# hku-mars/loam_livox

Hardware: AMD Instinct MI355X
Metric: scans_per_s (higher is better)
Workload: dtype f32 points / f64 solve; 1 GPU; C2: 24k-pt Mid-40 scan vs 5M-pt corner+surface map, 10 ICP iters (fixed), k=5, Q-full; scan_points=24000, map_points=4975193, map_corner=995155, map_surf=3980038, icp_iters=10, distinct_scans_in_batch=256

## Files before the change

### loam_livox_amd/build.py

```python
from __future__ import annotations

import os
import shutil
import subprocess
import sys

HERE = os.path.dirname(os.path.abspath(__file__))
CSRC = os.path.join(HERE, "csrc")
LIB = os.environ.get("LL_LIB_OUT") or os.path.join(HERE, "libloamlivox_hip.so")
SOURCES = ["ll_api_common.hip", "ll_api_fe.hip", "ll_api_map.hip", "ll_api_reg.hip", "ll_api_voxel.hip", "ll_api_cellmap.hip", "ll_api_scene_align.hip", "ll_api_keyframe_bank.hip", "ll_api_pose_graph.hip", "ll_api_history.hip", "ll_api_history_batch_buffer.hip", "ll_api_history_batch_stores.hip", "ll_api_history_batch_extract.hip", "ll_api_history_batch_cells.hip", "ll_fe_kernels.hip", "ll_map_kernels.hip", "ll_reg_query_kernels.hip", "ll_reg_solve_kernels.hip", "ll_reg_maps_kernels.hip", "ll_reg_aux_kernels.hip", "ll_reg_small_kernels.hip", "ll_knn_kernels.hip", "ll_voxel_kernels.hip", "ll_cellmap_kernels.hip", "ll_cellmap_extract_kernels.hip", "ll_cellmap_select_kernels.hip", "ll_spin_kernels.hip", "ll_spin_api.hip", "ll_history_batch_kernels.hip", "ll_cellmap_batch_kernels.hip", "ll_cellmap_batch_extract_kernels.hip", "ll_cellmatch_batch_kernels.hip", "ll_fullmap_batch_kernels.hip", "ll_keyframe_bank_kernels.hip", "ll_pose_graph_kernels.hip"]
HEADERS = ["ll_api_internal.h", "ll_api_history_batch_internal.h", "ll_device.h", "ll_fe_core.h", "ll_knn_core.h", "ll_knn_coop.h", "ll_knn_tile.h", "ll_reg_query.h", "ll_reg_solve_fast.h", "ll_reg_big_path.h", "ll_reg_solve_general.h", "ll_reg_solve_common.h", "ll_reg_small_solve.h", "ll_reg_core.h", "ll_voxel.h", "ll_voxel_core.h", "ll_cellmap.h", "ll_cellmap_core.h", "ll_cellmap_select_core.h", "ll_spin.h", "ll_spin_core.h", "ll_history_batch.h", "ll_cellmap_batch.h", "ll_cellmap_batch_core.h", "ll_cellmap_batch_extract_core.h", "ll_cellmatch_batch.h", "ll_cellmatch_batch_core.h", "ll_fullmap_batch.h", "ll_fullmap_batch_core.h", "ll_keyframe_bank.h", "ll_keyframe_bank_core.h", "ll_pose_graph.h", "ll_pose_graph_core.h", "../../include/loam_livox_hip.h"]
FLAGS = ["--offload-arch=gfx950", "-O3", "-std=c++17", "-fPIC", "-ffp-contract=off", "-Wno-unused-result"]
FLAGS += os.environ.get("LL_EXTRA_HIPCC_FLAGS", "").split()


def hipcc() -> str:
    for cand in (shutil.which("hipcc"), "/opt/rocm/bin/hipcc"):
        if cand and os.path.exists(cand):
            return cand
    raise RuntimeError("hipcc not found (ROCm toolchain required to build libloamlivox_hip.so)")



def needs_build(lib: str = LIB) -> bool:
    if not os.path.exists(lib):
        return True
    t = os.path.getmtime(lib)
    deps = [os.path.join(CSRC, f) for f in SOURCES + HEADERS] + [os.path.abspath(__file__)]
    return any(os.path.getmtime(d) > t for d in deps)


def build(force: bool = False, verbose: bool = False, lib: str = LIB, extra_flags=()) -> str:
    if not force and not needs_build(lib):
        return lib
    cc = hipcc()
    default = os.path.join(HERE, "libloamlivox_hip.so")
    objdir = os.path.join(HERE, "build" if lib == default else "build_" + os.path.basename(lib).replace(".so", ""))
    os.makedirs(objdir, exist_ok=True)
    objs = []
    procs = []
    for src in SOURCES:
        obj = os.path.join(objdir, src.replace(".hip", ".o"))
        cmd = [cc] + FLAGS + list(extra_flags) + ["-c", os.path.join(CSRC, src), "-o", obj]
        if verbose:
            print(" ".join(cmd), file=sys.stderr)
        procs.append((src, subprocess.Popen(cmd, stdout=subprocess.PIPE, stderr=subprocess.STDOUT)))
        objs.append(obj)
    for src, p in procs:
        out, _ = p.communicate()
        if p.returncode != 0:
            raise RuntimeError(f"hipcc failed on {src}:\n{out.decode()}")
        if verbose and out:
            print(out.decode(), file=sys.stderr)
    cmd = [cc, "--offload-arch=gfx950", "-shared", "-fPIC", "-o", lib] + objs
    subprocess.check_call(cmd)
    return lib


if __name__ == "__main__":
    print(build(force="--force" in sys.argv, verbose=True))
```

### loam_livox_amd/csrc/ll_reg_solve_fast.h

```cpp
#pragma once
#include <hip/hip_runtime.h>

#include "ll_reg_query.h"
#include "ll_reg_solve_common.h"

namespace ll {

#define RS_WAVES (RS_THREADS / 64)

#define LL_CTX_DECL(x)                                   \
    double R_[9], t_[3];                                  \
    MbRot mb_;                                            \
    {                                                     \
        const double q_[4] = {(x)[0], (x)[1], (x)[2], (x)[3]}; \
        quat_to_mat(q_, R_);                              \
        t_[0] = (x)[4];                                   \
        t_[1] = (x)[5];                                   \
        t_[2] = (x)[6];                                   \
        if (DEBLUR) mb_prepare(q_, mb_);                  \
    }
#define LL_CTX_ACCUM(kind, ff, a, v, huber_a, acc)                                                        \
    do {                                                                                                  \
        const double f_[3] = {(double)(ff).x, (double)(ff).y, (double)(ff).z};                            \
        if (DEBLUR)                                                                                       \
            block_accumulate_mb((kind), mb_, t_, (double)(ff).w, f_, (a), (v), (huber_a), (acc));  \
        else                                                                                              \
            block_accumulate((kind), R_, t_, f_, (a), (v), (huber_a), (acc));            \
    } while (0)
#define LL_CTX_L1(out, kind, ff, a, v, huber_a, q_last)                                                   \
    do {                                                                                                  \
        const double f_[3] = {(double)(ff).x, (double)(ff).y, (double)(ff).z};                            \
        if (DEBLUR)                                                                                       \
            (out) = block_l1_mb((kind), mb_, t_, (double)(ff).w, f_, (a), (v), (huber_a), (q_last));      \
        else                                                                                              \
            (out) = block_l1((kind), R_, t_, f_, (a), (v), (huber_a), (q_last));                          \
    } while (0)

#ifdef LL_SOLVE_TIMING
#define LL_T0(var) long long var = clock64()
#define LL_TACC(slot, var)                                   \
    do {                                                     \
        if (threadIdx.x == 0) sh.tcyc[slot] += clock64() - var; \
    } while (0)
#else
#define LL_T0(var)
#define LL_TACC(slot, var)
#endif

struct SolveShared {
    long long tcyc[16];
    LmCtl ctl;
    double red[RS_WAVES][LL_NACC];
    double sum[LL_NACC];
    int need;
    int hist[256];
    int sel_bin, sel_cnt, n_cand;
    int isum[RS_WAVES];
    unsigned long long lsum[RS_WAVES];
    unsigned long long sel_prefix;
    int sel_rank;
    int n_active, n_corner_avail, n_surf_avail, n_unique;
    int l1_valid;
    int pt_T, pt_Tl, pt_kc, pt_priv;
    double fit[10];
    int pt_nl;
    double thr;
    int grp_g, grp_G, grp_seq, grp_abort;
    int xch_seq, xch_epoch;
    unsigned int xch[LL_GRP][2 * LL_NACC];
};

#define LL_GRP_SPIN_LIMIT (1 << 22)
template <bool FULL>
__device__ __forceinline__ void group_barrier(const RegDev &rd, int b, SolveShared &sh)
{
    if (FULL) __threadfence();
    __syncthreads();
    if (threadIdx.x == 0 && !sh.grp_abort) {
        const int target = (++sh.grp_seq) * sh.grp_G;
        int *bar = rd.grp_ctl + 1 + 2 * b, *abt = bar + 1;
        __hip_atomic_fetch_add(bar, 1, __ATOMIC_RELEASE, __HIP_MEMORY_SCOPE_AGENT);
        int spins = 0;
        while (__hip_atomic_load(bar, __ATOMIC_RELAXED, __HIP_MEMORY_SCOPE_AGENT) < target) {
            if (++spins > LL_GRP_SPIN_LIMIT || ((spins & 1023) == 0 && __hip_atomic_load(abt, __ATOMIC_RELAXED, __HIP_MEMORY_SCOPE_AGENT))) {
                sh.grp_abort = 1;
                __hip_atomic_store(abt, 1, __ATOMIC_RELAXED, __HIP_MEMORY_SCOPE_AGENT);
                break;
            }
        }
        if (!sh.grp_abort && __hip_atomic_load(abt, __ATOMIC_RELAXED, __HIP_MEMORY_SCOPE_AGENT)) sh.grp_abort = 1;
    }
    __syncthreads();
    if (FULL) __threadfence();
}

template <bool FULL>
__device__ __forceinline__ void group_reduce(const RegDev &rd, int b, SolveShared &sh)
{
    const int tid = threadIdx.x, G = sh.grp_G;
    if (FULL) {
        double *part = rd.grp_part + ((size_t)b * 2 + (sh.grp_seq & 1)) * LL_GRP * LL_NACC;
        if (tid < LL_NACC) __hip_atomic_store(part + sh.grp_g * LL_NACC + tid, sh.sum[tid], __ATOMIC_RELAXED, __HIP_MEMORY_SCOPE_AGENT);
        group_barrier<true>(rd, b, sh);
        if (tid < LL_NACC) {
            double t = 0.0;
            for (int k = 0; k < G; k++) t += __hip_atomic_load(part + k * LL_NACC + tid, __ATOMIC_RELAXED, __HIP_MEMORY_SCOPE_AGENT);
            sh.sum[tid] = t;
        }
        __syncthreads();
        return;
    }
    constexpr int NG = 2 * LL_NACC;
    static_assert(LL_GRP * NG <= RS_THREADS, "one polling thread per granule");
    if (tid == 0) sh.xch_seq++;
    __syncthreads();
    const int seq = sh.xch_seq;
    if (!sh.grp_abort && seq < 4096) {
        const unsigned int tag = ((unsigned int)sh.xch_epoch << 12) | (unsigned int)seq;
        unsigned long long *slot = rd.grp_xch + ((size_t)b * 2 + (seq & 1)) * LL_GRP * NG;
        if (tid < NG) {
            const unsigned long long bits = (unsigned long long)__double_as_longlong(sh.sum[tid >> 1]);
            const unsigned int half = (tid & 1) ? (unsigned int)(bits >> 32) : (unsigned int)bits;
            __hip_atomic_store(slot + sh.grp_g * NG + tid, ((unsigned long long)tag << 32) | (unsigned long long)half, __ATOMIC_RELAXED,
                               __HIP_MEMORY_SCOPE_AGENT);
        }
        if (tid < G * NG) {
            const int *abt = rd.grp_ctl + 2 + 2 * b;
            unsigned long long v = __hip_atomic_load(slot + tid, __ATOMIC_RELAXED, __HIP_MEMORY_SCOPE_AGENT);
            int spins = 0;
            while ((unsigned int)(v >> 32) != tag) {
                if (++spins > LL_GRP_SPIN_LIMIT || ((spins & 1023) == 0 && __hip_atomic_load(abt, __ATOMIC_RELAXED, __HIP_MEMORY_SCOPE_AGENT))) {
                    sh.grp_abort = 1;
                    __hip_atomic_store(const_cast<int *>(abt), 1, __ATOMIC_RELAXED, __HIP_MEMORY_SCOPE_AGENT);
                    break;
                }
                __builtin_amdgcn_s_sleep(1);
                v = __hip_atomic_load(slot + tid, __ATOMIC_RELAXED, __HIP_MEMORY_SCOPE_AGENT);
            }
            sh.xch[tid / NG][tid % NG] = (unsigned int)v;
        }
    } else if (tid == 0 && !sh.grp_abort) {
        sh.grp_abort = 1;
        __hip_atomic_store(rd.grp_ctl + 2 + 2 * b, 1, __ATOMIC_RELAXED, __HIP_MEMORY_SCOPE_AGENT);
    }
    __syncthreads();
    if (tid < LL_NACC && !sh.grp_abort) {
        double t = 0.0;
        for (int k = 0; k < G; k++)
            t += __longlong_as_double((long long)(((unsigned long long)sh.xch[k][2 * tid + 1] << 32) | (unsigned long long)sh.xch[k][2 * tid]));
        sh.sum[tid] = t;
    }
    __syncthreads();
}

__device__ __forceinline__ unsigned long long block_sum_u64(unsigned long long v, SolveShared &sh)
{
    const int tid = threadIdx.x, lane = tid & 63, wave = tid >> 6;
#pragma unroll
    for (int off = 32; off > 0; off >>= 1) v += (unsigned long long)__shfl_down((long long)v, off);
    if (lane == 0) sh.lsum[wave] = v;
    __syncthreads();
    unsigned long long s = 0;
    for (int w = 0; w < RS_WAVES; w++) s += sh.lsum[w];
    __syncthreads();
    return s;
}

__device__ int block_sum_int(int v, SolveShared &sh)
{
    const int tid = threadIdx.x, lane = tid & 63, wave = tid >> 6;
#pragma unroll
    for (int off = 32; off > 0; off >>= 1) v += __shfl_down(v, off);
    if (lane == 0) sh.isum[wave] = v;
    __syncthreads();
    int s = 0;
    for (int w = 0; w < RS_WAVES; w++) s += sh.isum[w];
    __syncthreads();
    return s;
}

__device__ __forceinline__ unsigned long long hash64(unsigned long long k)
{
    k ^= k >> 33;
    k *= 0xff51afd7ed558ccdull;
    k ^= k >> 33;
    k *= 0xc4ceb9fe1a85ec53ull;
    k ^= k >> 33;
    return k;
}



#define FAST_MAXK (FAST_MAX_BLOCKS / RS_THREADS)
#define HASH_EMPTY 0xffffffffffffffffull
#define HT_SIZE 16384
#define HT_PART 6144
#define DD2_WORDS 16384
#define DD2_SLOTS (DD2_WORDS * 16)
#define DD2B_WORDS 8192
#define DD2B_SLOTS (DD2B_WORDS * 16)
#define DD2_LIST 2048
#define SEL_BINS 4096
#define SEL_CAND 1024


template <int NK>
__device__ __forceinline__ void inlier_threshold_regs(const double (&l1r)[NK], int total, unsigned long long *s_table, SolveShared &sh,
                                                      const RegConst &rc)
{
    static_assert(NK <= 64 && NK <= FAST_MAXK, "register tile of the fast paths (one bit per entry in the 64-bit masks)");
    const int tid = threadIdx.x;
    LL_T0(t_dd);
    unsigned long long first_mask = 0;
    {
        int my = 0;
        unsigned int *bmA = (unsigned int *)s_table;
        unsigned int *bmB = bmA + DD2_WORDS;
        unsigned long long *dl = (unsigned long long *)(bmB + DD2B_WORDS);
        {
            uint4 *z = (uint4 *)s_table;
            for (int e = tid; e < (DD2_WORDS + DD2B_WORDS) / 4; e += RS_THREADS) z[e] = make_uint4(0u, 0u, 0u, 0u);
            if (tid == 0) sh.n_cand = 0;
        }
        __syncthreads();
        const int kt = (total + RS_THREADS - 1) / RS_THREADS;
        auto slot_a = [](unsigned long long key) -> unsigned int {
            unsigned int h = (unsigned int)key * 0x9E3779B1u;
            h ^= h >> 15;
            h += (unsigned int)(key >> 32) * 0x85EBCA77u;
            h ^= h >> 13;
            return h & (DD2_SLOTS - 1);
        };
        auto slot_b = [](unsigned long long key) -> unsigned int {
            unsigned int h2 = ((unsigned int)(key >> 32) * 0xC2B2AE3Du) ^ ((unsigned int)key * 0x27D4EB2Fu);
            return (h2 ^ (h2 >> 16)) & (DD2B_SLOTS - 1);
        };
        unsigned long long valid_mask = 0, cont_mask = 0;
#pragma unroll
        for (int k = 0; k < NK; k++) {
            if (k >= kt) continue;
            const double l1 = l1r[k];
            const bool valid = l1 >= 0.0;
            const unsigned int slot = slot_a((unsigned long long)__double_as_longlong(l1));
            const unsigned int bit0 = valid ? (1u << ((slot & 15u) * 2u)) : 0u;
            const unsigned int old = atomicOr(&bmA[slot >> 4], bit0);
            atomicOr(&bmA[slot >> 4], (old & bit0) << 1);
            if (valid) valid_mask |= 1ull << k;
        }
        __syncthreads();
#pragma unroll
        for (int k = 0; k < NK; k++) {
            if (k >= kt) continue;
            const unsigned long long key = (unsigned long long)__double_as_longlong(l1r[k]);
            const unsigned int slot = slot_a(key);
            const bool contested = ((valid_mask >> k) & 1ull) && ((bmA[slot >> 4] >> ((slot & 15u) * 2u)) & 2u);
            const unsigned int h2 = slot_b(key);
            const unsigned int bit0 = contested ? (1u << ((h2 & 15u) * 2u)) : 0u;
            const unsigned int old = atomicOr(&bmB[h2 >> 4], bit0);
            atomicOr(&bmB[h2 >> 4], (old & bit0) << 1);
            if (contested) cont_mask |= 1ull << k;
        }
        __syncthreads();
        unsigned long long twice_mask = 0;
#pragma unroll
        for (int k = 0; k < NK; k++) {
            if (k >= kt) continue;
            const unsigned int h2 = slot_b((unsigned long long)__double_as_longlong(l1r[k]));
            if (((cont_mask >> k) & 1ull) && ((bmB[h2 >> 4] >> ((h2 & 15u) * 2u)) & 2u)) twice_mask |= 1ull << k;
        }
        my = __popcll(valid_mask & ~twice_mask);
        first_mask = valid_mask & ~twice_mask;
        int my_pos[2] = {-1, -1};
        int n_twice = __popcll(twice_mask);
        if (twice_mask) {
            int got = 0;
#pragma unroll
            for (int k = 0; k < NK; k++) {
                if (!((twice_mask >> k) & 1ull)) continue;
                const int pos = atomicAdd(&sh.n_cand, 1);
                if (pos < DD2_LIST) dl[pos] = (unsigned long long)__double_as_longlong(l1r[k]);
                if (got < 2) my_pos[got] = pos;
                got++;
            }
        }
        const int over = block_sum_int(n_twice > 2 ? 1 : 0, sh);
        const int n_list = sh.n_cand;
        if (n_list <= DD2_LIST && over == 0) {
            if (twice_mask) {
                int got = 0;
#pragma unroll
                for (int k = 0; k < NK; k++) {
                    if (!((twice_mask >> k) & 1ull)) continue;
                    const int pos = my_pos[got < 2 ? got : 1];
                    got++;
                    const unsigned long long key = (unsigned long long)__double_as_longlong(l1r[k]);
                    bool dup = false;
                    for (int j = 0; j < pos; j++) dup |= (dl[j] == key);
                    if (!dup) {
                        first_mask |= 1ull << k;
                        my++;
                    }
                }
            }
        } else {
            first_mask = 0;
            my = 0;
            const int rounds = (total + HT_PART - 1) / HT_PART;
            for (int rnd = 0; rnd < rounds; rnd++) {
                __syncthreads();
                for (int e = tid; e < HT_SIZE; e += RS_THREADS) s_table[e] = HASH_EMPTY;
                __syncthreads();
#pragma unroll
                for (int k = 0; k < NK; k++) {
                    const double l1 = l1r[k];
                    if (!(l1 >= 0.0)) continue;
                    const unsigned long long key = (unsigned long long)__double_as_longlong(l1);
                    const unsigned long long hk = hash64(key);
                    if ((int)((hk >> 40) % (unsigned long long)rounds) != rnd) continue;
                    unsigned int h = (unsigned int)hk & (HT_SIZE - 1);
                    for (;;) {
                        const unsigned long long old = atomicCAS(&s_table[h], HASH_EMPTY, key);
                        if (old == HASH_EMPTY) {
                            first_mask |= (1ull << k);
                            my++;
                            break;
                        }
                        if (old == key) break;
                        h = (h + 1u) & (HT_SIZE - 1);
                    }
                }
            }
        }
        const int nu = block_sum_int(my, sh);
        if (tid == 0) {
            sh.n_unique = nu;
            sh.sel_prefix = 0ull;
            int target = (int)(rc.inlier_ratio * (double)nu);
            if (target > nu - 1) target = nu - 1;
            sh.sel_rank = target;
        }
        __syncthreads();
    }
    LL_TACC(3, t_dd);
    LL_T0(t_sel);
    if (sh.n_unique > 0) {
        int *bins = (int *)s_table;
        unsigned long long *cand = s_table + SEL_BINS / 2;
        double kmin = INFINITY, kmax = -INFINITY;
#pragma unroll
        for (int k = 0; k < NK; k++)
            if (first_mask & (1ull << k)) {
                kmin = fmin(kmin, l1r[k]);
                kmax = fmax(kmax, l1r[k]);
            }
        for (int off = 32; off > 0; off >>= 1) {
            kmin = fmin(kmin, __shfl_down(kmin, off));
            kmax = fmax(kmax, __shfl_down(kmax, off));
        }
        if ((tid & 63) == 0) {
            sh.red[tid >> 6][0] = kmin;
            sh.red[tid >> 6][1] = kmax;
        }
        for (int e = tid; e < SEL_BINS; e += RS_THREADS) bins[e] = 0;
        __syncthreads();
        double lo = sh.red[0][0], hi = sh.red[0][1];
        for (int w = 1; w < RS_WAVES; w++) {
            lo = fmin(lo, sh.red[w][0]);
            hi = fmax(hi, sh.red[w][1]);
        }
        const double scale = (hi > lo) ? (double)(SEL_BINS - 1) / (hi - lo) : 0.0;
#pragma unroll
        for (int k = 0; k < NK; k++)
            if (first_mask & (1ull << k)) {
                int bi = (int)((l1r[k] - lo) * scale);
                bi = bi < 0 ? 0 : (bi > SEL_BINS - 1 ? SEL_BINS - 1 : bi);
                atomicAdd(&bins[bi], 1);
            }
        __syncthreads();
        {
            const int per = SEL_BINS / RS_THREADS;
            const int lane = tid & 63, wave = tid >> 6;
            int part = 0;
            for (int e = 0; e < per; e++) part += bins[tid * per + e];
            int incl = part;
#pragma unroll
            for (int off = 1; off < 64; off <<= 1) {
                const int y = __shfl_up(incl, off);
                if (lane >= off) incl += y;
            }
            if (lane == 63) sh.isum[wave] = incl;
            if (tid == 0) sh.n_cand = 0;
            __syncthreads();
            int below = incl - part;
            for (int w = 0; w < wave; w++) below += sh.isum[w];
            const int rank = sh.sel_rank;
            __syncthreads();
            const bool last_thread = tid == RS_THREADS - 1;
            if ((rank >= below && rank < below + part) || (last_thread && rank >= below + part)) {
                int cum = below, bi = tid * per;
                for (; bi < tid * per + per - 1; bi++) {
                    if (cum + bins[bi] > rank) break;
                    cum += bins[bi];
                }
                sh.sel_bin = bi;
                sh.sel_rank = rank - cum;
                sh.sel_cnt = bins[bi];
            }
            __syncthreads();
        }
        if (sh.sel_cnt <= SEL_CAND) {
            const int sel_bin = sh.sel_bin;
#pragma unroll
            for (int k = 0; k < NK; k++)
                if (first_mask & (1ull << k)) {
                    int bi = (int)((l1r[k] - lo) * scale);
                    bi = bi < 0 ? 0 : (bi > SEL_BINS - 1 ? SEL_BINS - 1 : bi);
                    if (bi == sel_bin) cand[atomicAdd(&sh.n_cand, 1)] = (unsigned long long)__double_as_longlong(l1r[k]);
                }
            __syncthreads();
            const int m = sh.n_cand;
            for (int i = tid; i < m; i += RS_THREADS) {
                const unsigned long long ki = cand[i];
                int rk = 0;
                for (int j = 0; j < m; j++) rk += (cand[j] < ki) ? 1 : 0;
                if (rk == sh.sel_rank) sh.sel_prefix = ki;
            }
            __syncthreads();
        } else {
            const int sel_bin = sh.sel_bin;
            if (tid == 0) sh.sel_prefix = 0ull;
            __syncthreads();
            for (int pass = 0; pass < 8; pass++) {
                const int shift = 56 - 8 * pass;
                for (int e = tid; e < 256; e += RS_THREADS) sh.hist[e] = 0;
                __syncthreads();
                const unsigned long long prefix = sh.sel_prefix;
#pragma unroll
                for (int k = 0; k < NK; k++) {
                    if (!(first_mask & (1ull << k))) continue;
                    int bi = (int)((l1r[k] - lo) * scale);
                    bi = bi < 0 ? 0 : (bi > SEL_BINS - 1 ? SEL_BINS - 1 : bi);
                    if (bi != sel_bin) continue;
                    const unsigned long long key = (unsigned long long)__double_as_longlong(l1r[k]);
                    if (pass == 0 || (key >> (shift + 8)) == prefix) atomicAdd(&sh.hist[(int)((key >> shift) & 255ull)], 1);
                }
                __syncthreads();
                if (tid == 0) {
                    int rank = sh.sel_rank, d = 0, cum = 0;
                    for (d = 0; d < 256; d++) {
                        if (cum + sh.hist[d] > rank) break;
                        cum += sh.hist[d];
                    }
                    if (d > 255) d = 255;
                    sh.sel_rank = rank - cum;
                    sh.sel_prefix = (prefix << 8) | (unsigned long long)d;
                }
                __syncthreads();
            }
        }
        if (tid == 0) sh.thr = fmax(rc.inliner_dis, __longlong_as_double((long long)sh.sel_prefix));
    } else {
        if (tid == 0) sh.thr = rc.inliner_dis;
    }
    __syncthreads();
    LL_TACC(4, t_sel);
}

struct BlkRegs {
    float4 f;
    double a0, a1, a2, v0, v1, v2;
};

__device__ __forceinline__ void load_blk(const RegDev &rd, size_t sb, const double *av, int slot, BlkRegs &r)
{
    r.f = gload_f4(rd.blk_f + sb + slot);
    av_load(av, rd.cap, slot, slot < rd.cap_c, r.a0, r.a1, r.a2, r.v0, r.v1, r.v2);
}


#define PT_SLOTS 8192
#define PT_MAX_PROBE 192
#define PT_LDS_BYTES 155648
#define PT_TCAP (PT_LDS_BYTES / 32)
#define LL_LINE_CACHE_MAX 1024
#define PT_EMPTY_A 0xffffffffffffffffull
#define PT_EMPTY_B 0xffffffffu
#define PT_PRIVATE 0xffffu
#define PT_INACTIVE 0xfffeu
#define PT_NTRIP (FAST_MAX_BLOCKS / RS_THREADS / 8)

struct PtSlot {
    unsigned long long a;
    unsigned int b;
    unsigned int id;
};

__device__ __forceinline__ unsigned short gload_u16(const unsigned short *p) { return *(const LL_AS_GLOBAL unsigned short *)p; }

__device__ __forceinline__ unsigned int pt_hash(unsigned int p0, unsigned int p1, unsigned int p2)
{
    unsigned int h = p0 * 0x9E3779B1u;
    h ^= h >> 15;
    h += p1 * 0x85EBCA77u;
    h ^= h >> 13;
    h += p2 * 0xC2B2AE3Du;
    h ^= h >> 16;
    return h;
}

template <int MAX_PROBE = PT_MAX_PROBE>
__device__ __forceinline__ unsigned int pt_insert(LL_AS_LDS PtSlot *ht, unsigned int p0, unsigned int p1, unsigned int p2)
{
    const unsigned long long A = ((unsigned long long)p0 << 32) | (unsigned long long)p1;
    const unsigned int hh = pt_hash(p0, p1, p2);
    unsigned int h = hh & (PT_SLOTS - 1);
    const unsigned int step = ((hh >> 13) | 1u) & (PT_SLOTS - 1);
    for (int probe = 0; probe < MAX_PROBE; probe++) {
        unsigned long long a = __hip_atomic_load(&ht[h].a, __ATOMIC_RELAXED, __HIP_MEMORY_SCOPE_WORKGROUP);
        unsigned int bb = __hip_atomic_load(&ht[h].b, __ATOMIC_RELAXED, __HIP_MEMORY_SCOPE_WORKGROUP);
        if (a == A && bb == p2) return h;
        if (a == PT_EMPTY_A) {
            if (__hip_atomic_compare_exchange_strong(&ht[h].a, &a, A, __ATOMIC_RELAXED, __ATOMIC_RELAXED, __HIP_MEMORY_SCOPE_WORKGROUP)) a = A;
        }
        if (a == A) {
            if (bb == PT_EMPTY_B) {
                if (__hip_atomic_compare_exchange_strong(&ht[h].b, &bb, p2, __ATOMIC_RELAXED, __ATOMIC_RELAXED, __HIP_MEMORY_SCOPE_WORKGROUP)) bb = p2;
            }
            if (bb == p2) return h;
        }
        h = (h + step) & (PT_SLOTS - 1);
    }
    return PT_PRIVATE;
}

template <bool SCALED = false>
__device__ __forceinline__ void pt_plane(const f4 *map_pts, const double *pose_last, unsigned int i0, unsigned int i1, unsigned int i2, int4 &ob, int4 &oc)
{
    const f4 m0 = gload_pt(map_pts + i0), m1 = gload_pt(map_pts + i1), m2 = gload_pt(map_pts + i2);
    const double pa[3] = {(double)m0.x, (double)m0.y, (double)m0.z};
    const double pb[3] = {(double)m1.x, (double)m1.y, (double)m1.z};
    const double pc[3] = {(double)m2.x, (double)m2.y, (double)m2.z};
    double a_out[3] = {0.0, 0.0, 0.0}, v_out[3] = {0.0, 0.0, 0.0};
    (void)block_plane(pose_last, pa, pb, pc, a_out, v_out);
    if (SCALED) {
        double m_[3], beta_;
        plane_scale(v_out, a_out[0], m_, &beta_);
        v_out[0] = m_[0], v_out[1] = m_[1], v_out[2] = m_[2], a_out[0] = beta_;
    }
    ob = make_int4(__double2loint(v_out[0]), __double2hiint(v_out[0]), __double2loint(v_out[1]), __double2hiint(v_out[1]));
    oc = make_int4(__double2loint(v_out[2]), __double2hiint(v_out[2]), __double2loint(a_out[0]), __double2hiint(a_out[0]));
}

__device__ __forceinline__ int4 *pt_table_global(const RegDev &rd, int b, int g, bool grouped)
{
    return rd.pl_tab + ((size_t)b * rd.tab_cap + (grouped ? (size_t)g * (rd.tab_cap / LL_GRP) : 0)) * 2;
}

#define PT_MAP_OFF (PT_SLOTS * 16)
template <bool GROUPED>
__device__ __noinline__ unsigned long long census_and_plane_table(const RegDev &rd, const RegConst &rc, const f4 *map_pts, int b, const RegState *st,
                                                                  int nC, int nS, uint4 *s_raw, SolveShared &sh)
{
    const int tid = threadIdx.x, lane = tid & 63, wave = tid >> 6;
    constexpr int G = GROUPED ? LL_GRP : 1, GS = G * RS_THREADS;
    const int g = GROUPED ? sh.grp_g : 0;
    const int p0 = g * RS_THREADS + tid;
// ... 538 lines not shown
        }
        __syncthreads();
        LL_TACC(1, t1);
    }
}

template <int NK, bool GROUPED>
__device__ __noinline__ unsigned long long inlier_phase3(const RegDev &rd, const RegConst &rc, int b, RegState *st, SolveShared &sh, uint4 *s_raw,
                                                         unsigned long long act, int nC, int nS)
{
    constexpr int DEBLUR = 0;
    const int tid = threadIdx.x;
    const int nSp = (nS + RS_THREADS - 1) / RS_THREADS * RS_THREADS;
    const int totp = nSp + nC;
    const size_t sb = (size_t)b * rd.cap;
    LL_T0(t_l1);
    double *l1g = rd.blk_l1 + sb;
    if (!sh.l1_valid) {
        LL_CTX_DECL(sh.ctl.x)
        constexpr int G = GROUPED ? LL_GRP : 1, GS = G * RS_THREADS;
        const int g = GROUPED ? sh.grp_g : 0;
        const int p0 = g * RS_THREADS + tid;
        const int4 *tabG = pt_table_global(rd, b, g, GROUPED);
        const unsigned short *ids = rd.blk_id + (size_t)b * rd.cap_s;
        const float4 *feat = rd.surf_feat + (size_t)b * rd.feat_stride_s;
        const double *av = rd.blk_av + (size_t)b * 6 * rd.cap;
        int k = 0;
        for (int p = p0; p < nS; p += GS, k++) {
            if (!((act >> (g + G * k)) & 1ull)) continue;
            const float4 ff = gload_f4(feat + p);
            const unsigned int id = gload_u16(ids + p);
            const int4 qb = gload_i4(tabG + 2 * id), qc = gload_i4(tabG + 2 * id + 1);
            const double f[3] = {(double)ff.x, (double)ff.y, (double)ff.z};
            const double v[3] = {__hiloint2double(qb.y, qb.x), __hiloint2double(qb.w, qb.z), __hiloint2double(qc.y, qc.x)};
            l1g[rd.cap_c + p] = plane_l1_scaled(R_, t_, f, v, __hiloint2double(qc.w, qc.z), rc.huber_a, st->pose_last);
        }
        const int kpl = nSp / RS_THREADS;
        k = 0;
        for (int l = p0; l < nC; l += GS, k++) {
            if (!((act >> (kpl + g + G * k)) & 1ull)) continue;
            BlkRegs br;
            load_blk(rd, sb, av, l, br);
            const double a[3] = {br.a0, br.a1, br.a2};
            const double v[3] = {br.v0, br.v1, br.v2};
            double l1;
            LL_CTX_L1(l1, BLK_LINE, br.f, a, v, rc.huber_a, st->pose_last);
            l1g[l] = l1;
        }
        if (GROUPED)
            group_barrier<true>(rd, b, sh);
        else
            __syncthreads();
    } else if (tid == 0) {
        sh.tcyc[9] += 1;
    }
    double l1r[NK];
    {
        const int kt = (totp + RS_THREADS - 1) / RS_THREADS;
#pragma unroll
        for (int k = 0; k < NK; k++) {
            const int j = tid + k * RS_THREADS;
            double v = -1.0;
            if (k < kt) {
                const int jc = j < totp ? j : 0;
                const size_t src = jc < nS ? (size_t)rd.cap_c + jc : (jc >= nSp ? (size_t)(jc - nSp) : (size_t)rd.cap_c);
                v = gload_f64(l1g + src);
            }
            l1r[k] = v;
        }
#pragma unroll
        for (int k = 0; k < NK; k++) l1r[k] = ((act >> k) & 1ull) ? l1r[k] : -1.0;
    }
    __syncthreads();
    LL_TACC(2, t_l1);

    inlier_threshold_regs<NK>(l1r, totp, (unsigned long long *)s_raw, sh, rc);

    LL_T0(t_prune);
    {
        const double thr = sh.thr;
        int na = 0;
#pragma unroll
        for (int k = 0; k < NK; k++) {
            if (!((act >> k) & 1ull)) continue;
            if (l1r[k] > thr)
                act &= ~(1ull << k);
            else
                na++;
        }
        na = block_sum_int(na, sh);
        if (tid == 0) sh.n_active = na;
        __syncthreads();
    }
    LL_TACC(7, t_prune);
    return act;
}

template <bool GROUPED>
__device__ void solve_fast3(const RegDev &rd, const RegConst &rc, const f4 *map_pts, int b, RegState *st, SolveShared &sh, uint4 *s_raw)
{
    constexpr int DEBLUR = 0;
    const int tid = threadIdx.x;
    const int nC = rd.n_corner[b], nS = rd.n_surf[b];
    const int nSp = (nS + RS_THREADS - 1) / RS_THREADS * RS_THREADS;
    const int totp = nSp + nC;
    const size_t sb = (size_t)b * rd.cap;
    if (tid < 16) sh.tcyc[tid] = 0;
    __syncthreads();
    LL_T0(t_total);

    unsigned long long act = census_and_plane_table<GROUPED>(rd, rc, map_pts, b, st, nC, nS, s_raw, sh);

    solver_lm3<true, GROUPED>(rd, rc, b, nC, nS, st->inc, rc.ceres_prerun_times, sh.n_active, act, s_raw, st->pose_last, sh);
    int lm_iters = sh.ctl.iteration;

    if (totp <= 36 * RS_THREADS)
        act = inlier_phase3<36, GROUPED>(rd, rc, b, st, sh, s_raw, act, nC, nS);
    else
        act = inlier_phase3<FAST_MAXK, GROUPED>(rd, rc, b, st, sh, s_raw, act, nC, nS);

    {
        __shared__ double x_start_3[7];
        if (tid < 7) x_start_3[tid] = sh.ctl.x[tid];
        plane_table_reload(rd, b, GROUPED, s_raw, sh);
        solver_lm3<false, GROUPED>(rd, rc, b, nC, nS, x_start_3, rc.ceres_max_iterations, sh.n_active, act, s_raw, st->pose_last, sh);
    }
    lm_iters += sh.ctl.iteration;
    if (GROUPED) {
        group_barrier<false>(rd, b, sh);
        if (sh.grp_g != 0) return;
        if (sh.grp_abort) {
            if (tid == 0) {
                st->aborted = 1;
                st->done = 1;
                st->icp_iters += 1;
            }
            return;
        }
    }
    solve_epilogue(rc, st, sh, lm_iters);
#ifdef LL_SOLVE_TIMING
    LL_TACC(5, t_total);
    if (tid == 0)
        for (int i = 0; i < 16; i++) st->dbg_cycles[i] += sh.tcyc[i];
#endif
}

struct SolveTicket {
    int b, g, G;
};
__device__ __forceinline__ SolveTicket solve_fast_ticket(const RegDev &rd, const RegConst &rc, SolveShared &sh)
{
    SolveTicket t = {(int)blockIdx.x, 0, 1};
    if (rc.solve_group > 1) {
        if (threadIdx.x == 0) sh.grp_seq = atomicAdd(rd.grp_ctl, 1);
        __syncthreads();
        t.G = rc.solve_group;
        t.b = sh.grp_seq / t.G;
        t.g = sh.grp_seq - t.b * t.G;
        __syncthreads();
    }
    return t;
}
__device__ __forceinline__ bool solve_fast_check(const RegDev &rd, const RegConst &rc, int b, int g, int nC, int nS, RegState *st)
{
    if (padded_block_count(nC, nS) > FAST_MAX_BLOCKS || !scan_is_compact(rd, rc, b)) {
        if (g == 0 && threadIdx.x == 0) {
            st->aborted = 1;
            st->done = 1;
            st->icp_iters += 1;
        }
// ... 19 lines not shown
```

Baseline: 52620 scans/s.

## Fuse inlier histogram build into dedup pass and batch LDS atomics branchlessly

Computes the min/max range before de-duplication and builds the selection histogram during the first slot-table pass, subtracting duplicates afterward instead of re-binning unique values in a separate pass. This removes a reduction, a zeroing pass and several block barriers. The dedup and candidate-gather loops are restructured into batches of independent LDS atomics with dummy no-op targets so the divergent branches become predicated code, and the per-thread twice-list handling is simplified. The histogram range now covers duplicate values too, and the extra no-op atomics add LDS traffic.

```diff
diff --git a/loam_livox_amd/build.py b/loam_livox_amd/build.py
--- a/loam_livox_amd/build.py
+++ b/loam_livox_amd/build.py
@@ -9,7 +9,7 @@
 CSRC = os.path.join(HERE, "csrc")
 LIB = os.environ.get("LL_LIB_OUT") or os.path.join(HERE, "libloamlivox_hip.so")
 SOURCES = ["ll_api_common.hip", "ll_api_fe.hip", "ll_api_map.hip", "ll_api_reg.hip", "ll_api_voxel.hip", "ll_api_cellmap.hip", "ll_api_scene_align.hip", "ll_api_keyframe_bank.hip", "ll_api_pose_graph.hip", "ll_api_history.hip", "ll_api_history_batch_buffer.hip", "ll_api_history_batch_stores.hip", "ll_api_history_batch_extract.hip", "ll_api_history_batch_cells.hip", "ll_fe_kernels.hip", "ll_map_kernels.hip", "ll_reg_query_kernels.hip", "ll_reg_solve_kernels.hip", "ll_reg_maps_kernels.hip", "ll_reg_aux_kernels.hip", "ll_reg_small_kernels.hip", "ll_knn_kernels.hip", "ll_voxel_kernels.hip", "ll_cellmap_kernels.hip", "ll_cellmap_extract_kernels.hip", "ll_cellmap_select_kernels.hip", "ll_spin_kernels.hip", "ll_spin_api.hip", "ll_history_batch_kernels.hip", "ll_cellmap_batch_kernels.hip", "ll_cellmap_batch_extract_kernels.hip", "ll_cellmatch_batch_kernels.hip", "ll_fullmap_batch_kernels.hip", "ll_keyframe_bank_kernels.hip", "ll_pose_graph_kernels.hip"]
-HEADERS = ["ll_api_internal.h", "ll_api_history_batch_internal.h", "ll_device.h", "ll_fe_core.h", "ll_knn_core.h", "ll_knn_coop.h", "ll_knn_tile.h", "ll_reg_query.h", "ll_reg_solve_fast.h", "ll_reg_big_path.h", "ll_reg_solve_general.h", "ll_reg_solve_common.h", "ll_reg_small_solve.h", "ll_reg_core.h", "ll_voxel.h", "ll_voxel_core.h", "ll_cellmap.h", "ll_cellmap_core.h", "ll_cellmap_select_core.h", "ll_spin.h", "ll_spin_core.h", "ll_history_batch.h", "ll_cellmap_batch.h", "ll_cellmap_batch_core.h", "ll_cellmap_batch_extract_core.h", "ll_cellmatch_batch.h", "ll_cellmatch_batch_core.h", "ll_fullmap_batch.h", "ll_fullmap_batch_core.h", "ll_keyframe_bank.h", "ll_keyframe_bank_core.h", "ll_pose_graph.h", "ll_pose_graph_core.h", "../../include/loam_livox_hip.h"]
+HEADERS = ["ll_api_internal.h", "ll_api_history_batch_internal.h", "ll_device.h", "ll_fe_core.h", "ll_knn_core.h", "ll_knn_coop.h", "ll_knn_tile.h", "ll_reg_query.h", "ll_reg_solve_fast.h", "ll_reg_big_path.h", "ll_reg_solve_general.h", "ll_reg_solve_common.h", "ll_inlier_slots.h", "ll_reg_small_solve.h", "ll_reg_core.h", "ll_voxel.h", "ll_voxel_core.h", "ll_cellmap.h", "ll_cellmap_core.h", "ll_cellmap_select_core.h", "ll_spin.h", "ll_spin_core.h", "ll_history_batch.h", "ll_cellmap_batch.h", "ll_cellmap_batch_core.h", "ll_cellmap_batch_extract_core.h", "ll_cellmatch_batch.h", "ll_cellmatch_batch_core.h", "ll_fullmap_batch.h", "ll_fullmap_batch_core.h", "ll_keyframe_bank.h", "ll_keyframe_bank_core.h", "ll_pose_graph.h", "ll_pose_graph_core.h", "../../include/loam_livox_hip.h"]
 FLAGS = ["--offload-arch=gfx950", "-O3", "-std=c++17", "-fPIC", "-ffp-contract=off", "-Wno-unused-result"]
 FLAGS += os.environ.get("LL_EXTRA_HIPCC_FLAGS", "").split()
 
diff --git a/loam_livox_amd/csrc/ll_inlier_slots.h b/loam_livox_amd/csrc/ll_inlier_slots.h
--- /dev/null
+++ b/loam_livox_amd/csrc/ll_inlier_slots.h
@@ -0,0 +1,55 @@
+#pragma once
+#include <stdint.h>
+
+#ifndef LL_HD
+#if defined(__HIPCC__)
+#define LL_HD __host__ __device__ __forceinline__
+#else
+#define LL_HD inline
+#endif
+#endif
+
+namespace ll {
+
+#define DD2_WORDS 16384
+#define DD2_SLOTS (DD2_WORDS * 16)
+#define DD2B_WORDS 8192
+#define DD2B_SLOTS (DD2B_WORDS * 16)
+#define DD2_LIST_CAP 2048
+#define SEL_BINS 4096
+#define SEL_CAND 1024
+
+LL_HD unsigned int dd2_slot_a(unsigned long long key)
+{
+    unsigned int h = (unsigned int)key * 0x9E3779B1u;
+    h ^= h >> 15;
+    h += (unsigned int)(key >> 32) * 0x85EBCA77u;
+    h ^= h >> 13;
+    return h & (DD2_SLOTS - 1);
+}
+
+LL_HD unsigned int dd2_slot_b(unsigned long long key)
+{
+    const unsigned int h2 = ((unsigned int)(key >> 32) * 0xC2B2AE3Du) ^ ((unsigned int)key * 0x27D4EB2Fu);
+    return (h2 ^ (h2 >> 16)) & (DD2B_SLOTS - 1);
+}
+
+LL_HD unsigned int dd2_word(unsigned int slot) { return slot >> 4; }
+LL_HD unsigned int dd2_shift(unsigned int slot) { return (slot & 15u) * 2u; }
+LL_HD unsigned int dd2_first(unsigned int slot, bool takes_part) { return takes_part ? (1u << dd2_shift(slot)) : 0u; }
+LL_HD unsigned int dd2_second(unsigned int old_word, unsigned int first) { return (old_word & first) << 1; }
+LL_HD bool dd2_contested(unsigned int word, unsigned int slot) { return ((word >> dd2_shift(slot)) & 2u) != 0u; }
+
+LL_HD double sel_scale(double lo, double hi) { return (hi > lo) ? (double)(SEL_BINS - 1) / (hi - lo) : 0.0; }
+LL_HD int sel_bin_of(double v, double lo, double scale)
+{
+    const int bi = (int)((v - lo) * scale);
+    return bi < 0 ? 0 : (bi > SEL_BINS - 1 ? SEL_BINS - 1 : bi);
+}
+LL_HD int sel_target_rank(double ratio, int n_distinct)
+{
+    const int target = (int)(ratio * (double)n_distinct);
+    return target > n_distinct - 1 ? n_distinct - 1 : target;
+}
+
+}
diff --git a/loam_livox_amd/csrc/ll_reg_solve_fast.h b/loam_livox_amd/csrc/ll_reg_solve_fast.h
--- a/loam_livox_amd/csrc/ll_reg_solve_fast.h
+++ b/loam_livox_amd/csrc/ll_reg_solve_fast.h
@@ -1,6 +1,7 @@
 #pragma once
 #include <hip/hip_runtime.h>
 
+#include "ll_inlier_slots.h"
 #include "ll_reg_query.h"
 #include "ll_reg_solve_common.h"
 
@@ -55,6 +56,7 @@
     int need;
     int hist[256];
     int sel_bin, sel_cnt, n_cand;
+    int dd_over;
     int isum[RS_WAVES];
     unsigned long long lsum[RS_WAVES];
     unsigned long long sel_prefix;
@@ -166,7 +168,7 @@
     return s;
 }
 
-__device__ int block_sum_int(int v, SolveShared &sh)
+__device__ __forceinline__ int block_sum_int_inl(int v, SolveShared &sh)
 {
     const int tid = threadIdx.x, lane = tid & 63, wave = tid >> 6;
 #pragma unroll
@@ -178,6 +180,8 @@
     __syncthreads();
     return s;
 }
+
+__device__ int block_sum_int(int v, SolveShared &sh) { return block_sum_int_inl(v, sh); }
 
 __device__ __forceinline__ unsigned long long hash64(unsigned long long k)
 {
@@ -195,13 +199,10 @@
 #define HASH_EMPTY 0xffffffffffffffffull
 #define HT_SIZE 16384
 #define HT_PART 6144
-#define DD2_WORDS 16384
-#define DD2_SLOTS (DD2_WORDS * 16)
-#define DD2B_WORDS 8192
-#define DD2B_SLOTS (DD2B_WORDS * 16)
 #define DD2_LIST 2048
-#define SEL_BINS 4096
-#define SEL_CAND 1024
+static_assert(DD2_LIST == DD2_LIST_CAP, "the list capacity the host protocol is run with");
+#define DD2_BATCH 12
+#define SEL_BINS_OFF (HT_SIZE * 8)
 
 
 template <int NK>
@@ -212,93 +213,150 @@
     const int tid = threadIdx.x;
     LL_T0(t_dd);
     unsigned long long first_mask = 0;
+    int *bins = (int *)((char *)s_table + SEL_BINS_OFF);
+    double lo, hi, scale;
+    int nu;
     {
         int my = 0;
         unsigned int *bmA = (unsigned int *)s_table;
         unsigned int *bmB = bmA + DD2_WORDS;
         unsigned long long *dl = (unsigned long long *)(bmB + DD2B_WORDS);
+        static_assert((DD2_WORDS + DD2B_WORDS) * 4 + DD2_LIST * 8 <= SEL_BINS_OFF, "slot tables and list lie below the histogram");
+        static_assert(NK % DD2_BATCH == 0 && RS_THREADS <= DD2B_WORDS && RS_THREADS <= SEL_BINS, "whole batches; a no-op word per thread");
         {
+            double kmin = INFINITY, kmax = -INFINITY;
+#pragma unroll
+            for (int k = 0; k < NK; k++) {
+                const bool valid = l1r[k] >= 0.0;
+                kmin = valid ? fmin(kmin, l1r[k]) : kmin;
+                kmax = valid ? fmax(kmax, l1r[k]) : kmax;
+            }
+            for (int off = 32; off > 0; off >>= 1) {
+                kmin = fmin(kmin, __shfl_down(kmin, off));
+                kmax = fmax(kmax, __shfl_down(kmax, off));
+            }
+            if ((tid & 63) == 0) {
+                sh.red[tid >> 6][0] = kmin;
+                sh.red[tid >> 6][1] = kmax;
+            }
             uint4 *z = (uint4 *)s_table;
             for (int e = tid; e < (DD2_WORDS + DD2B_WORDS) / 4; e += RS_THREADS) z[e] = make_uint4(0u, 0u, 0u, 0u);
-            if (tid == 0) sh.n_cand = 0;
+            z = (uint4 *)(bins);
+            for (int e = tid; e < SEL_BINS / 4; e += RS_THREADS) z[e] = make_uint4(0u, 0u, 0u, 0u);
+            if (tid == 0) sh.n_cand = 0, sh.dd_over = 0;
         }
         __syncthreads();
+        lo = sh.red[0][0], hi = sh.red[0][1];
+        for (int w = 1; w < RS_WAVES; w++) {
+            lo = fmin(lo, sh.red[w][0]);
+            hi = fmax(hi, sh.red[w][1]);
+        }
+        scale = sel_scale(lo, hi);
         const int kt = (total + RS_THREADS - 1) / RS_THREADS;
-        auto slot_a = [](unsigned long long key) -> unsigned int {
-            unsigned int h = (unsigned int)key * 0x9E3779B1u;
-            h ^= h >> 15;
-            h += (unsigned int)(key >> 32) * 0x85EBCA77u;
-            h ^= h >> 13;
-            return h & (DD2_SLOTS - 1);
-        };
-        auto slot_b = [](unsigned long long key) -> unsigned int {
-            unsigned int h2 = ((unsigned int)(key >> 32) * 0xC2B2AE3Du) ^ ((unsigned int)key * 0x27D4EB2Fu);
-            return (h2 ^ (h2 >> 16)) & (DD2B_SLOTS - 1);
-        };
         unsigned long long valid_mask = 0, cont_mask = 0;
 #pragma unroll
-        for (int k = 0; k < NK; k++) {
-            if (k >= kt) continue;
-            const double l1 = l1r[k];
-            const bool valid = l1 >= 0.0;
-            const unsigned int slot = slot_a((unsigned long long)__double_as_longlong(l1));
-            const unsigned int bit0 = valid ? (1u << ((slot & 15u) * 2u)) : 0u;
-            const unsigned int old = atomicOr(&bmA[slot >> 4], bit0);
-            atomicOr(&bmA[slot >> 4], (old & bit0) << 1);
-            if (valid) valid_mask |= 1ull << k;
+        for (int k0 = 0; k0 < NK; k0 += DD2_BATCH) {
+            if (k0 >= kt) continue;
+            unsigned int w[DD2_BATCH], b0[DD2_BATCH], old[DD2_BATCH], hb[DD2_BATCH];
+#pragma unroll
+            for (int i = 0; i < DD2_BATCH; i++) {
+                const double l1 = l1r[k0 + i];
+                const bool valid = l1 >= 0.0;
+                const unsigned int slot = dd2_slot_a((unsigned long long)__double_as_longlong(l1));
+                w[i] = valid ? dd2_word(slot) : (unsigned int)tid;
+                b0[i] = dd2_first(slot, valid);
+                hb[i] = valid ? (unsigned int)sel_bin_of(l1, lo, scale) : (unsigned int)tid;
+                if (valid) valid_mask |= 1ull << (k0 + i);
+            }
+#pragma unroll
+            for (int i = 0; i < DD2_BATCH; i++) old[i] = atomicOr(&bmA[w[i]], b0[i]);
+#pragma unroll
+            for (int i = 0; i < DD2_BATCH; i++) atomicOr(&bmA[w[i]], dd2_second(old[i], b0[i]));
+#pragma unroll
+            for (int i = 0; i < DD2_BATCH; i++) atomicAdd(&bins[hb[i]], (int)((valid_mask >> (k0 + i)) & 1ull));
         }
         __syncthreads();
 #pragma unroll
-        for (int k = 0; k < NK; k++) {
-            if (k >= kt) continue;
-            const unsigned long long key = (unsigned long long)__double_as_longlong(l1r[k]);
-            const unsigned int slot = slot_a(key);
-            const bool contested = ((valid_mask >> k) & 1ull) && ((bmA[slot >> 4] >> ((slot & 15u) * 2u)) & 2u);
-            const unsigned int h2 = slot_b(key);
-            const unsigned int bit0 = contested ? (1u << ((h2 & 15u) * 2u)) : 0u;
-            const unsigned int old = atomicOr(&bmB[h2 >> 4], bit0);
-            atomicOr(&bmB[h2 >> 4], (old & bit0) << 1);
-            if (contested) cont_mask |= 1ull << k;
+        for (int k0 = 0; k0 < NK; k0 += DD2_BATCH) {
+            if (k0 >= kt) continue;
+            unsigned int w[DD2_BATCH], b0[DD2_BATCH], old[DD2_BATCH];
+#pragma unroll
+            for (int i = 0; i < DD2_BATCH; i++) {
+                const unsigned int slot = dd2_slot_a((unsigned long long)__double_as_longlong(l1r[k0 + i]));
+                old[i] = bmA[dd2_word(slot)];
+            }
+#pragma unroll
+            for (int i = 0; i < DD2_BATCH; i++) {
+                const unsigned long long key = (unsigned long long)__double_as_longlong(l1r[k0 + i]);
+                const bool contested = ((valid_mask >> (k0 + i)) & 1ull) && dd2_contested(old[i], dd2_slot_a(key));
+                const unsigned int h2 = dd2_slot_b(key);
+                w[i] = contested ? dd2_word(h2) : (unsigned int)tid;
+                b0[i] = dd2_first(h2, contested);
+                if (contested) cont_mask |= 1ull << (k0 + i);
+            }
+#pragma unroll
+            for (int i = 0; i < DD2_BATCH; i++) old[i] = atomicOr(&bmB[w[i]], b0[i]);
+#pragma unroll
+            for (int i = 0; i < DD2_BATCH; i++) atomicOr(&bmB[w[i]], dd2_second(old[i], b0[i]));
         }
         __syncthreads();
         unsigned long long twice_mask = 0;
 #pragma unroll
-        for (int k = 0; k < NK; k++) {
-            if (k >= kt) continue;
-            const unsigned int h2 = slot_b((unsigned long long)__double_as_longlong(l1r[k]));
-            if (((cont_mask >> k) & 1ull) && ((bmB[h2 >> 4] >> ((h2 & 15u) * 2u)) & 2u)) twice_mask |= 1ull << k;
+        for (int k0 = 0; k0 < NK; k0 += DD2_BATCH) {
+            if (k0 >= kt) continue;
+            unsigned int rd2[DD2_BATCH];
+#pragma unroll
+            for (int i = 0; i < DD2_BATCH; i++) rd2[i] = bmB[dd2_word(dd2_slot_b((unsigned long long)__double_as_longlong(l1r[k0 + i])))];
+#pragma unroll
+            for (int i = 0; i < DD2_BATCH; i++) {
+                const unsigned int h2 = dd2_slot_b((unsigned long long)__double_as_longlong(l1r[k0 + i]));
+                if (((cont_mask >> (k0 + i)) & 1ull) && dd2_contested(rd2[i], h2)) twice_mask |= 1ull << (k0 + i);
+            }
         }
         my = __popcll(valid_mask & ~twice_mask);
         first_mask = valid_mask & ~twice_mask;
-        int my_pos[2] = {-1, -1};
-        int n_twice = __popcll(twice_mask);
+        const int n_twice = __popcll(twice_mask);
+        const int i0 = n_twice > 0 ? __ffsll((long long)twice_mask) - 1 : -1;
+        const unsigned long long rest = twice_mask & (twice_mask - 1ull);
+        const int i1 = n_twice > 1 ? __ffsll((long long)rest) - 1 : -1;
+        double tv0 = 0.0, tv1 = 0.0;
+        int base = 0;
         if (twice_mask) {
-            int got = 0;
 #pragma unroll
             for (int k = 0; k < NK; k++) {
-                if (!((twice_mask >> k) & 1ull)) continue;
-                const int pos = atomicAdd(&sh.n_cand, 1);
-                if (pos < DD2_LIST) dl[pos] = (unsigned long long)__double_as_longlong(l1r[k]);
-                if (got < 2) my_pos[got] = pos;
-                got++;
-            }
-        }
-        const int over = block_sum_int(n_twice > 2 ? 1 : 0, sh);
+                tv0 = (k == i0) ? l1r[k] : tv0;
+                tv1 = (k == i1) ? l1r[k] : tv1;
+            }
+            base = atomicAdd(&sh.n_cand, n_twice);
+            if (base < DD2_LIST) dl[base] = (unsigned long long)__double_as_longlong(tv0);
+            if (n_twice > 1 && base + 1 < DD2_LIST) dl[base + 1] = (unsigned long long)__double_as_longlong(tv1);
+        }
+        if (n_twice > 2) sh.dd_over = 1;
+        __syncthreads();
+        const int over = sh.dd_over;
         const int n_list = sh.n_cand;
         if (n_list <= DD2_LIST && over == 0) {
             if (twice_mask) {
-                int got = 0;
-#pragma unroll
-                for (int k = 0; k < NK; k++) {
-                    if (!((twice_mask >> k) & 1ull)) continue;
-                    const int pos = my_pos[got < 2 ? got : 1];
-                    got++;
-                    const unsigned long long key = (unsigned long long)__double_as_longlong(l1r[k]);
-                    bool dup = false;
-                    for (int j = 0; j < pos; j++) dup |= (dl[j] == key);
-                    if (!dup) {
-                        first_mask |= 1ull << k;
+                const unsigned long long key0 = (unsigned long long)__double_as_longlong(tv0), key1 = (unsigned long long)__double_as_longlong(tv1);
+                bool dup0 = false, dup1 = false;
+                for (int j = 0; j < base; j++) {
+                    const unsigned long long e = dl[j];
+                    dup0 |= (e == key0);
+                    dup1 |= (e == key1);
+                }
+                dup1 |= (key1 == key0);
+                if (!dup0) {
+                    first_mask |= 1ull << i0;
+                    my++;
+                } else {
+                    atomicAdd(&bins[sel_bin_of(tv0, lo, scale)], -1);
+                }
+                if (n_twice > 1) {
+                    if (!dup1) {
+                        first_mask |= 1ull << i1;
                         my++;
+                    } else {
+                        atomicAdd(&bins[sel_bin_of(tv1, lo, scale)], -1);
                     }
                 }
             }
@@ -310,10 +368,11 @@
                 __syncthreads();
                 for (int e = tid; e < HT_SIZE; e += RS_THREADS) s_table[e] = HASH_EMPTY;
                 __syncthreads();
-#pragma unroll
-                for (int k = 0; k < NK; k++) {
-                    const double l1 = l1r[k];
-                    if (!(l1 >= 0.0)) continue;
+                for (unsigned long long rem = valid_mask; rem; rem &= rem - 1ull) {
+                    const int kk = __ffsll((long long)rem) - 1;
+                    double l1 = 0.0;
+#pragma unroll
+                    for (int k = 0; k < NK; k++) l1 = (k == kk) ? l1r[k] : l1;
                     const unsigned long long key = (unsigned long long)__double_as_longlong(l1);
                     const unsigned long long hk = hash64(key);
                     if ((int)((hk >> 40) % (unsigned long long)rounds) != rnd) continue;
@@ -321,67 +380,40 @@
                     for (;;) {
                         const unsigned long long old = atomicCAS(&s_table[h], HASH_EMPTY, key);
                         if (old == HASH_EMPTY) {
-                            first_mask |= (1ull << k);
+                            first_mask |= (1ull << kk);
                             my++;
                             break;
                         }
-                        if (old == key) break;
+                        if (old == key) {
+                            atomicAdd(&bins[sel_bin_of(l1, lo, scale)], -1);
+                            break;
+                        }
                         h = (h + 1u) & (HT_SIZE - 1);
                     }
                 }
             }
         }
-        const int nu = block_sum_int(my, sh);
+        nu = block_sum_int_inl(my, sh);
         if (tid == 0) {
             sh.n_unique = nu;
             sh.sel_prefix = 0ull;
-            int target = (int)(rc.inlier_ratio * (double)nu);
-            if (target > nu - 1) target = nu - 1;
-            sh.sel_rank = target;
-        }
-        __syncthreads();
+        }
     }
     LL_TACC(3, t_dd);
     LL_T0(t_sel);
-    if (sh.n_unique > 0) {
-        int *bins = (int *)s_table;
-        unsigned long long *cand = s_table + SEL_BINS / 2;
-        double kmin = INFINITY, kmax = -INFINITY;
-#pragma unroll
-        for (int k = 0; k < NK; k++)
-            if (first_mask & (1ull << k)) {
-                kmin = fmin(kmin, l1r[k]);
-                kmax = fmax(kmax, l1r[k]);
-            }
-        for (int off = 32; off > 0; off >>= 1) {
-            kmin = fmin(kmin, __shfl_down(kmin, off));
-            kmax = fmax(kmax, __shfl_down(kmax, off));
-        }
-        if ((tid & 63) == 0) {
-            sh.red[tid >> 6][0] = kmin;
-            sh.red[tid >> 6][1] = kmax;
-        }
-        for (int e = tid; e < SEL_BINS; e += RS_THREADS) bins[e] = 0;
-        __syncthreads();
-        double lo = sh.red[0][0], hi = sh.red[0][1];
-        for (int w = 1; w < RS_WAVES; w++) {
-            lo = fmin(lo, sh.red[w][0]);
-            hi = fmax(hi, sh.red[w][1]);
-        }
-        const double scale = (hi > lo) ? (double)(SEL_BINS - 1) / (hi - lo) : 0.0;
-#pragma unroll
-        for (int k = 0; k < NK; k++)
-            if (first_mask & (1ull << k)) {
-                int bi = (int)((l1r[k] - lo) * scale);
-                bi = bi < 0 ? 0 : (bi > SEL_BINS - 1 ? SEL_BINS - 1 : bi);
-                atomicAdd(&bins[bi], 1);
-            }
-        __syncthreads();
+    if (nu > 0) {
+        unsigned long long *cand = s_table;
+        unsigned long long *dump = s_table + SEL_CAND;
+        static_assert((SEL_CAND + RS_THREADS) * 8 <= SEL_BINS_OFF, "candidates lie below the histogram");
         {
             const int per = SEL_BINS / RS_THREADS;
             const int lane = tid & 63, wave = tid >> 6;
+            static_assert(per == 8, "a thread's bins are two 16-byte reads");
+            const uint4 q0 = ((const uint4 *)(bins + tid * per))[0], q1 = ((const uint4 *)(bins + tid * per))[1];
+            const int c[per] = {(int)q0.x, (int)q0.y, (int)q0.z, (int)q0.w, (int)q1.x, (int)q1.y, (int)q1.z, (int)q1.w};
             int part = 0;
-            for (int e = 0; e < per; e++) part += bins[tid * per + e];
+#pragma unroll
+            for (int e = 0; e < per; e++) part += c[e];
             int incl = part;
 #pragma unroll
             for (int off = 1; off < 64; off <<= 1) {
@@ -393,30 +425,40 @@
             __syncthreads();
             int below = incl - part;
             for (int w = 0; w < wave; w++) below += sh.isum[w];
-            const int rank = sh.sel_rank;
-            __syncthreads();
+            const int rank = sel_target_rank(rc.inlier_ratio, nu);
             const bool last_thread = tid == RS_THREADS - 1;
             if ((rank >= below && rank < below + part) || (last_thread && rank >= below + part)) {
-                int cum = below, bi = tid * per;
-                for (; bi < tid * per + per - 1; bi++) {
-                    if (cum + bins[bi] > rank) break;
-                    cum += bins[bi];
+                int cum = below, sel = per - 1, cnt = c[per - 1];
+                bool found = false;
+#pragma unroll
+                for (int e = 0; e < per - 1; e++) {
+                    const bool here = !found && cum + c[e] > rank;
+                    sel = here ? e : sel;
+                    cnt = here ? c[e] : cnt;
+                    found = found || here;
+                    cum += found ? 0 : c[e];
                 }
-                sh.sel_bin = bi;
+                sh.sel_bin = tid * per + sel;
                 sh.sel_rank = rank - cum;
-                sh.sel_cnt = bins[bi];
+                sh.sel_cnt = cnt;
             }
             __syncthreads();
         }
         if (sh.sel_cnt <= SEL_CAND) {
             const int sel_bin = sh.sel_bin;
-#pragma unroll
-            for (int k = 0; k < NK; k++)
-                if (first_mask & (1ull << k)) {
-                    int bi = (int)((l1r[k] - lo) * scale);
-                    bi = bi < 0 ? 0 : (bi > SEL_BINS - 1 ? SEL_BINS - 1 : bi);
-                    if (bi == sel_bin) cand[atomicAdd(&sh.n_cand, 1)] = (unsigned long long)__double_as_longlong(l1r[k]);
-                }
+            unsigned long long cmask = 0;
+#pragma unroll
+            for (int k = 0; k < NK; k++) {
+                const bool is = ((first_mask >> k) & 1ull) && sel_bin_of(l1r[k], lo, scale) == sel_bin;
+                cmask |= is ? (1ull << k) : 0ull;
+            }
+            int cbase = 0;
+            if (cmask) cbase = atomicAdd(&sh.n_cand, __popcll(cmask));
+#pragma unroll
+            for (int k = 0; k < NK; k++) {
+                unsigned long long *dst = ((cmask >> k) & 1ull) ? cand + cbase + __popcll(cmask & ((1ull << k) - 1ull)) : dump + tid;
+                *dst = (unsigned long long)__double_as_longlong(l1r[k]);
+            }
             __syncthreads();
             const int m = sh.n_cand;
             for (int i = tid; i < m; i += RS_THREADS) {
@@ -437,12 +479,10 @@
                 const unsigned long long prefix = sh.sel_prefix;
 #pragma unroll
                 for (int k = 0; k < NK; k++) {
-                    if (!(first_mask & (1ull << k))) continue;
-                    int bi = (int)((l1r[k] - lo) * scale);
-                    bi = bi < 0 ? 0 : (bi > SEL_BINS - 1 ? SEL_BINS - 1 : bi);
-                    if (bi != sel_bin) continue;
                     const unsigned long long key = (unsigned long long)__double_as_longlong(l1r[k]);
-                    if (pass == 0 || (key >> (shift + 8)) == prefix) atomicAdd(&sh.hist[(int)((key >> shift) & 255ull)], 1);
+                    const bool in = ((first_mask >> k) & 1ull) && sel_bin_of(l1r[k], lo, scale) == sel_bin &&
+                                    (pass == 0 || (key >> (shift + 8)) == prefix);
+                    atomicAdd(&sh.hist[in ? (int)((key >> shift) & 255ull) : (tid & 255)], in ? 1 : 0);
                 }
                 __syncthreads();
                 if (tid == 0) {
@@ -482,6 +522,7 @@
 #define PT_MAX_PROBE 192
 #define PT_LDS_BYTES 155648
 #define PT_TCAP (PT_LDS_BYTES / 32)
+static_assert(SEL_BINS_OFF + SEL_BINS * 4 <= PT_LDS_BYTES, "inlier_threshold_regs: the histogram behind the de-duplication tables fits s_raw");
 #define LL_LINE_CACHE_MAX 1024
 #define PT_EMPTY_A 0xffffffffffffffffull
 #define PT_EMPTY_B 0xffffffffu
@@ -1186,11 +1227,9 @@
         int na = 0;
 #pragma unroll
         for (int k = 0; k < NK; k++) {
-            if (!((act >> k) & 1ull)) continue;
-            if (l1r[k] > thr)
-                act &= ~(1ull << k);
-            else
-                na++;
+            const bool on = (act >> k) & 1ull, out = on && l1r[k] > thr;
+            act &= out ? ~(1ull << k) : ~0ull;
+            na += (on && !out) ? 1 : 0;
         }
         na = block_sum_int(na, sh);
         if (tid == 0) sh.n_active = na;
```

Result: no change. 53080 scans/s, median of 6 (+0.9%).
